# danieleschmidt/DiffFE-Physics-Lab

Hardware: AMD Instinct MI355X
Metric: FEM solves/sec (fwd+adjoint), 2D P1 Poisson 1024^2 mesh, batch=256 per GPU (higher is better)
Workload: dtype f64

## Files before the change

difffe-physics-lab_amd/csrc/lattice.h:

```cpp
#pragma once
#include "common.h"

namespace diffhe_lattice __attribute__((visibility("hidden"))) {

using namespace diffhe;
typedef long long i64;

struct Level {
  int nx, ny, n, W, nd;
  const double* v;
  const float* v32;
  const _Float16* o16;
  const double* osc;
  const float* rd32;
  const float* mk32;
  const unsigned char* bc;
  const void* inv;
  const double* shift;
};

struct h16m {};
template <typename TM> struct MatTypes { typedef TM diag; typedef TM off; };
template <> struct MatTypes<h16m> { typedef float diag; typedef _Float16 off; };
__device__ __forceinline__ double ldc(const double* __restrict__ p, unsigned lv) { return p[lv]; }
__device__ __forceinline__ double ldc(const float* __restrict__ p, unsigned lv) { return (double)p[lv]; }
__device__ __forceinline__ double ldc(const _Float16* __restrict__ p, unsigned lv) { return (double)(float)p[lv]; }

__device__ inline double fast_rcp(double d) {
  const double r0 = __builtin_amdgcn_rcp(d);
  return fma(r0, fma(-d, r0, 1.0), r0);
}

// ... 180 lines not shown
    s.v[3] += (double)p.w;
  }
};

struct Src {
  rsrc_t r;
};
__device__ __forceinline__ Src make_src(const void* p) { return Src{make_rsrc(p)}; }
template <typename VT>
__device__ __forceinline__ VT ldsrc(const Src& s, unsigned voff, unsigned soff) { return VLane<VT>::ld(s.r, voff, soff); }

template <typename VT, bool SHARED> struct Coef;
template <typename VT> struct Coef<VT, true> {
  typedef float T;
  const float *v0, *v1, *v2, *v3, *rdp;
  __device__ __forceinline__ Coef(const Level& L, i64, unsigned, int) : v0(L.v32), v1(L.v32 + L.n), v2(L.v32 + 2 * (i64)L.n),
                                                                        v3(L.v32 + 3 * (i64)L.n), rdp(L.rd32) {}
  __device__ __forceinline__ T d(i64 i) const { return v0[i]; }
  __device__ __forceinline__ T e(i64 i) const { return v1[i]; }
  __device__ __forceinline__ T n2(i64 i) const { return v2[i]; }
  __device__ __forceinline__ T q3(i64 i) const { return v3[i]; }
  __device__ __forceinline__ T rd(i64 i, T) const { return rdp[i]; }
};
__device__ __forceinline__ float ldh(rsrc_t r, unsigned voff, float) {
  return (float)__builtin_bit_cast(_Float16, __builtin_amdgcn_raw_buffer_load_b16(r, voff, 0, 0));
}
__device__ __forceinline__ v2f ldh(rsrc_t r, unsigned voff, v2f) {
  typedef _Float16 h2 __attribute__((ext_vector_type(2)));
  const h2 h = __builtin_bit_cast(h2, __builtin_amdgcn_raw_buffer_load_b32(r, voff, 0, 0));
  return v2f{(float)h.x, (float)h.y};
}
__device__ __forceinline__ unsigned ldraw(rsrc_t r, unsigned voff, float) {
  return (unsigned)(unsigned short)__builtin_amdgcn_raw_buffer_load_b16(r, voff, 0, 0);
}
__device__ __forceinline__ unsigned ldraw(rsrc_t r, unsigned voff, v2f) {
  return (unsigned)__builtin_amdgcn_raw_buffer_load_b32(r, voff, 0, 0);
}
__device__ __forceinline__ float unraw(unsigned raw, float) { return (float)__builtin_bit_cast(_Float16, (unsigned short)raw); }
__device__ __forceinline__ v2f unraw(unsigned raw, v2f) {
  typedef _Float16 h2 __attribute__((ext_vector_type(2)));
  const h2 h = __builtin_bit_cast(h2, raw);
  return v2f{(float)h.x, (float)h.y};
}
template <typename VT> struct Coef<VT, false> {
  typedef VT T;
  rsrc_t r0, r1, r2, r3;
// ... 88 lines not shown
```

difffe-physics-lab_amd/csrc/lattice.hip:

```cpp
#include <stdlib.h>
#include <type_traits>
#include <string.h>

#include "lattice.h"

namespace diffhe_lattice __attribute__((visibility("hidden"))) {
namespace {

__global__ __launch_bounds__(256) void dia_apply_dot_kernel(Level L, int Bv, const double* __restrict__ scale,
                                                             const double* __restrict__ x, double* __restrict__ y,
                                                             double* __restrict__ part, int Bp) {
  __shared__ double lds[4 * kWave];
  const NodeMap nm = node_map(Bp);
  const int vb = Bv == 1 ? 0 : nm.b;
  double s = 0.0;
  for (int i = nm.node0; i < L.n; i += nm.stride) {
    const i64 o = (i64)i * Bp + nm.b;
    const double acc = row_scale(L, scale, i, nm.b) * dia_row(L, Bv, vb, x, i, nm.b, Bp) + shift_at(L, i) * x[o];
    y[o] = acc;
    s += acc * x[o];
  }
  STORE_PARTIAL(part, s);
}

// ... 1144 lines not shown
  if (launches) *launches = g_kp.n[id];
  return DIFFHE_OK;
}

static int fill_hier(Hier& H, const diffhe_mg_level* levels, int n_levels, int Bv, int Bp, const double* scale,
                     const double* omegas, int nu, int n_coarse) {
  if (!levels || n_levels < 1 || n_levels > kMaxLevels) return DIFFHE_E_BADARG;
  if (!diffhe::valid_batch_pad(Bp)) return DIFFHE_E_BATCHPAD;
  if (Bv != 1 && Bv != Bp) return DIFFHE_E_BADARG;
  if (nu < 1 || nu > 8 || n_coarse < 1 || !omegas) return DIFFHE_E_BADARG;
  for (int l = 0; l < n_levels; ++l) {
    const diffhe_mg_level& s = levels[l];
    if (s.nx < 2 || s.ny < 2 || (s.nd != 3 && s.nd != 4) || !s.vals || !s.is_bc) return DIFFHE_E_BADARG;
    if (l > 0) {
      const bool hx = levels[l - 1].nx == 2 * s.nx, hy = levels[l - 1].ny == 2 * s.ny;
      const bool kx = levels[l - 1].nx == s.nx, ky = levels[l - 1].ny == s.ny;
      if (!((hx && hy) || (hx && ky) || (kx && hy))) return DIFFHE_E_BADARG;
    }
    if ((long long)(s.nx + 1) * (s.ny + 1) > 0x7fffffffLL) return DIFFHE_E_TOOBIG;
    Level& L = H.lev[l];
    L.nx = s.nx; L.ny = s.ny; L.W = s.nx + 1; L.n = (s.nx + 1) * (s.ny + 1); L.nd = s.nd;
    L.v = s.vals; L.v32 = s.vals32; L.bc = s.is_bc; L.inv = s.dense_inv; L.shift = s.shift; L.rd32 = s.rdiag32; L.mk32 = s.mask32; L.o16 = (Bv == Bp && Bp > 1 && s.offdiag_scales) ? (const _Float16*)s.offdiag16 : nullptr;
    L.osc = s.offdiag_scales;
  }
  H.nl = n_levels; H.Bv = Bv; H.Bp = Bp; H.scale = scale; H.nu = nu; H.n_coarse = n_coarse;
  H.coarse_lmax = 2.0;
  H.fmg_coarse_cycles = 1;
  H.fuse = Bp % (2 * kWave) == 0 ? 2 : 1;
  H.pre4 = 1;
  H.dense_mfma = 1;
  for (int k = 0; k < 8; ++k) H.omega[k] = omegas[k < nu ? k : nu - 1];
  return DIFFHE_OK;
}

static long long carve(Hier& H, double* work, bool fp32) {
  long long off = 0;
  auto take = [&](long long cnt) {
    if (fp32) cnt = (cnt + 1) / 2;
    cnt = (cnt + 7) & ~7LL;
    double* p = work ? work + off : nullptr;
    off += cnt;
    return (void*)p;
  };
  for (int l = 0; l < H.nl; ++l) {
    const long long nb = (long long)H.lev[l].n * H.Bp;
    H.xa[l] = take(nb);
// ... 382 lines not shown
```

difffe-physics-lab_amd/csrc/lattice_fused.hip:

```cpp
#include "lattice.h"

namespace diffhe_lattice __attribute__((visibility("hidden"))) {
namespace {

template <typename VT, int ND, int CW, bool EDGE, bool SHARED>
__device__ __forceinline__ void fused_pre_body(const Level& L, VT ib, VT sb, const float* __restrict__ rhs,
                                               float* __restrict__ x2out, float* __restrict__ crhs, float w0, float w1,
                                               int cW, const unsigned char* __restrict__ cbc, int Bp, unsigned lb, int c0w,
                                               int r0, int r1) {
  constexpr int RW = 2 * CW + 1;
  constexpr int N1 = RW + 4, N2 = RW + 2;
  const int W = L.W, nyp = L.ny + 1;
  const i64 n = L.n;
  const VT Z = VLane<VT>::zero();
  typedef Coef<VT, SHARED> CF;
  i64 cbase = (i64)(r0 - 3) * W;
  if (cbase < 0) cbase = 0;
  const CF cf(L, cbase, lb, Bp);
  bool ok1[N1];
  unsigned off1[N1];
#pragma unroll
  for (int j = 0; j < N1; ++j) {
    int c = c0w - 2 + j;
    ok1[j] = !EDGE || (c >= 0 && c < W);
    if (EDGE) c = c < 0 ? 0 : (c > W - 1 ? W - 1 : c);
    off1[j] = 4u * ((unsigned)(c - (c0w - 2) + 2) * (unsigned)Bp + lb);
  }
  const i64 tile0 = ((i64)(r0 - 2) * W + (c0w - 4)) * Bp;
  const Src rr = make_src(rhs + tile0);
  const unsigned rowB = 4u * (unsigned)W * (unsigned)Bp;
  const float inv_w0 = 1.0f / w0;

  auto x1_row = [&](int R, VT* dst) {
    if (EDGE && (R < 0 || R >= nyp)) {
#pragma unroll
      for (int j = 0; j < N1; ++j) dst[j] = Z;
      return;
    }
    const unsigned sx = (unsigned)(R - (r0 - 2)) * rowB;
    const i64 rb = (i64)R * W + (c0w - 2);
// ... 230 lines not shown
template <typename VT, int ND, int CW, bool SHARED, int NW = 4, int MW = (SHARED ? 4 : 1)>
__global__ __launch_bounds__(64 * NW, MW) void fused_pre_kernel(Level L, const double* __restrict__ scale,
                                                         const float* __restrict__ rhs, float* __restrict__ x2out,
                                                         float* __restrict__ crhs, float w0, float w1, int cW,
                                                         const unsigned char* __restrict__ cbc, int Bp, int ncb, int TR) {
  constexpr int SPL = VLane<VT>::kSpl;
  const int lane = threadIdx.x & 63;
  const int wave = __builtin_amdgcn_readfirstlane(threadIdx.x >> 6);
  const unsigned lb = blockIdx.y * (SPL * kWave) + SPL * lane;
  const int tile = xcd_tile(blockIdx.x, gridDim.x);
  const int rc = tile / ncb, cb = tile - rc * ncb;
  const int nyp = L.ny + 1;
  const int J0 = (cb * NW + wave) * CW, I0 = rc * TR;
  const int cnyp = (nyp + 1) >> 1;
  const int I1 = (I0 + TR < cnyp) ? I0 + TR : cnyp;
  if (!(J0 < cW && I0 < I1)) return;
  const int c0w = 2 * J0 - 1;
  const int r0 = I0 > 0 ? 2 * I0 - 1 : 0;
  const int r1 = (2 * I1 < nyp) ? 2 * I1 : nyp;
  const VT sb = VLane<VT>::from_scale(scale, lb);
  const VT ib = 1.0f / sb;
  constexpr int RW = 2 * CW + 1;
  const bool edge = c0w - 2 < 0 || c0w + RW + 1 > L.W - 1 || r0 - 2 < 0 || r1 + 1 > nyp - 1;
  if (edge) fused_pre_body<VT, ND, CW, true, SHARED>(L, ib, sb, rhs, x2out, crhs, w0, w1, cW, cbc, Bp, lb, c0w, r0, r1);
  else fused_pre_body<VT, ND, CW, false, SHARED>(L, ib, sb, rhs, x2out, crhs, w0, w1, cW, cbc, Bp, lb, c0w, r0, r1);
}

template <typename VT, int ND, int RW, bool EDGE, bool DOT, bool SHARED, bool XZ>
__device__ __forceinline__ void fused_post_body(const Level& L, VT ib, const float* __restrict__ xin,
                                                const float* __restrict__ rhs, const float* __restrict__ ec,
                                                float* __restrict__ zout, float wA, float wB, int cW, int Bp, unsigned lb,
                                                int c0w, int r0, int r1, Acc& acc) {
  constexpr int N1 = RW + 4, N2 = RW + 2;
  constexpr int NCE = RW / 2 + 3;
  const int W = L.W, nyp = L.ny + 1;
  const i64 n = L.n;
  const VT Z = VLane<VT>::zero();
  typedef Coef<VT, SHARED> CF;
  i64 cbase = (i64)(r0 - 3) * W;
  if (cbase < 0) cbase = 0;
  const CF cf(L, cbase, lb, Bp);
  bool ok1[N1];
  unsigned off1[N1];
#pragma unroll
  for (int j = 0; j < N1; ++j) {
    int c = c0w - 2 + j;
    ok1[j] = !EDGE || (c >= 0 && c < W);
    if (EDGE) c = c < 0 ? 0 : (c > W - 1 ? W - 1 : c);
    off1[j] = 4u * ((unsigned)(c - (c0w - 2) + 2) * (unsigned)Bp + lb);
  }
  const int cj0 = (c0w >> 1) - 1;
  unsigned offc[NCE];
#pragma unroll
  for (int j = 0; j < NCE; ++j) {
    int cj = cj0 + j;
    cj = cj < 0 ? 0 : (cj > cW - 1 ? cW - 1 : cj);
    offc[j] = 4u * ((unsigned)cj * (unsigned)Bp + lb);
  }
  const i64 tile0 = ((i64)(r0 - 2) * W + (c0w - 4)) * Bp;
  const Src rx = make_src(XZ ? rhs + tile0 : xin + tile0);
  const Src rr = make_src(rhs + tile0);
  const int cr0 = (r0 - 2 > 0 ? r0 - 2 : 0) >> 1;
  const Src rc = make_src(ec + (i64)cr0 * cW * Bp);
// ... 3 lines not shown
    if (EDGE && (R < 0 || R >= nyp)) {
#pragma unroll
      for (int j = 0; j < N1; ++j) dst[j] = Z;
      return;
    }
    const unsigned sx = (unsigned)(R - (r0 - 2)) * rowB;
    const unsigned sc = (unsigned)((R >> 1) - cr0) * rowCB;
    VT ce[NCE], ce2[NCE];
#pragma unroll
    for (int j = 0; j < NCE; ++j) {
      ce[j] = ldsrc<VT>(rc, offc[j], sc);
      ce2[j] = (R & 1) ? ldsrc<VT>(rc, offc[j], sc + rowCB) : Z;
    }
    const i64 rb = (i64)R * W + (c0w - 2);
#pragma unroll
    for (int j = 0; j < N1; ++j) {
      VT corr;
      if (!(j & 1))
        corr = (R & 1) ? 0.5f * (ce[j / 2] + ce2[j / 2]) : ce[j / 2];
      else
        corr = (R & 1) ? 0.5f * (ce[(j + 1) / 2] + ce2[(j - 1) / 2]) : 0.5f * (ce[(j - 1) / 2] + ce[(j + 1) / 2]);
      i64 i = rb + j;
      if (EDGE) i = i < 0 ? 0 : (i > n - 1 ? n - 1 : i);
      const VT v = XZ ? L.mk32[i] * corr : ldsrc<VT>(rx, off1[j], sx) + L.mk32[i] * corr;
      dst[j] = ok1[j] ? v : Z;
    }
  };
  auto bu_row = [&](int R, VT* dst) {
    if (EDGE && (R < 0 || R >= nyp)) {
#pragma unroll
      for (int j = 0; j < N2; ++j) dst[j] = Z;
      return;
    }
    const unsigned sx = (unsigned)(R - (r0 - 2)) * rowB;
#pragma unroll
    for (int j = 0; j < N2; ++j) dst[j] = ok1[j + 1] ? ldsrc<VT>(rr, off1[j + 1], sx) * ib : Z;
  };
  auto x3_row = [&](int R, const VT* am, const VT* ac, const VT* ap, const VT* bu, VT* dst) {
    if (EDGE && (R < 0 || R >= nyp)) {
#pragma unroll
      for (int j = 0; j < N2; ++j) dst[j] = Z;
      return;
    }
    k1_row<VT, N2, ND, EDGE>(cf, n, W, R, c0w - 1, am, ac, ap, [&](int j, VT kx, typename CF::T, typename CF::T rd) {
      const VT v = ac[j + 1] + (wA * rd) * (bu[j] - kx);
      dst[j] = ok1[j + 1] ? v : Z;
    });
// ... 119 lines not shown
template <typename VT, int ND, int RW, bool DOT, bool SHARED, bool XZ = false, int NW = 4, int MW = (SHARED ? 4 : 1)>
__global__ __launch_bounds__(64 * NW, MW) void fused_post_kernel(Level L, const double* __restrict__ scale,
                                                          const float* __restrict__ xin, const float* __restrict__ rhs,
                                                          const float* __restrict__ ec, float* __restrict__ zout, float wA,
                                                          float wB, int cW, double* __restrict__ part, int Bp, int ncb,
                                                          int TR) {
  __shared__ double lds[NW * kWave];
  constexpr int SPL = VLane<VT>::kSpl;
  const int lane = threadIdx.x & 63;
  const int wave = __builtin_amdgcn_readfirstlane(threadIdx.x >> 6);
  const unsigned lb = blockIdx.y * (SPL * kWave) + SPL * lane;
  const int tile = xcd_tile(blockIdx.x, gridDim.x);
  const int rc = tile / ncb, cb = tile - rc * ncb;
  const int nyp = L.ny + 1;
  const int c0w = (cb * NW + wave) * RW;
  const int r0 = rc * TR;
  const int r1 = (r0 + TR < nyp) ? r0 + TR : nyp;
  const bool active = c0w < L.W && r0 < r1;
  const VT sb = VLane<VT>::from_scale(scale, lb);
  const VT ib = 1.0f / sb;
  Acc acc;
  if (active) {
    const bool edge = c0w - 2 < 0 || c0w + RW + 1 > L.W - 1 || r0 - 2 < 0 || r1 + 1 > nyp - 1;
    if (edge)
      fused_post_body<VT, ND, RW, true, DOT, SHARED, XZ>(L, ib, xin, rhs, ec, zout, wA, wB, cW, Bp, lb, c0w, r0, r1, acc);
    else
      fused_post_body<VT, ND, RW, false, DOT, SHARED, XZ>(L, ib, xin, rhs, ec, zout, wA, wB, cW, Bp, lb, c0w, r0, r1, acc);
  }
  if (DOT) {
#pragma unroll
    for (int q = 0; q < SPL; ++q) {
      const double f = scale ? scale[lb + q] : 1.0;
      const double t = block_sum_waves<NW>(acc.v[q] * f, lds);
      if (wave == 0) part[(i64)blockIdx.x * Bp + lb + q] = t;
    }
  }
}

}

void launch_fused_pre(const Level& L, const Level& C, int Bv, const double* scale, const float* rhs, float* x2, float* crhs,
                      double w0, double w1, int Bp, const StripGeom& g, int spl, hipStream_t st) {
  constexpr int CW = kRestrictCols;
  diffhe::account((9.0 + (Bv == 1 ? 0.0 : 4.0 + 2.0 * (L.nd - 1))) * (double)L.n * Bp);
  const dim3 grid(g.ncb * g.nrc, Bp / (spl * kWave));
#define FPRE(VT_, ND_, SH_)                                                                                               \
  hipLaunchKernelGGL((fused_pre_kernel<VT_, ND_, CW, SH_>), grid, dim3(256), 0, st, L, scale, rhs, x2, crhs,              \
                     (float)w0, (float)w1, C.W, C.bc, Bp, g.ncb, g.TR)
  if (Bv != 1) { if (L.nd == 3) FPRE(v2f, 3, false); else FPRE(v2f, 4, false); }
// ... 38 lines not shown
```

difffe-physics-lab_amd/diffhe/_hip.py:

```python
from __future__ import annotations

import ctypes as C
import os

import torch

_HERE = os.path.dirname(os.path.abspath(__file__))
LIB_PATH = os.environ.get("DIFFHE_HIP_LIB", os.path.join(os.path.dirname(_HERE), "lib", "libdiffhe_hip.so"))

_P, _I, _L, _D = C.c_void_p, C.c_int, C.c_longlong, C.c_double
ABI_VERSION = 8


class MgLevel(C.Structure):
    _fields_ = [("nx", _I), ("ny", _I), ("nd", _I), ("reserved", _I), ("vals", _P), ("is_bc", _P), ("vals32", _P),
                ("dense_inv", _P), ("shift", _P), ("rdiag32", _P), ("mask32", _P), ("offdiag16", _P), ("offdiag_scales", _P)]


_LV = C.POINTER(MgLevel)


class AmgLevel(C.Structure):
    _fields_ = [("n", _I), ("W", _I), ("vals", _P), ("cols", _P), ("agg", _P), ("agg_ptr", _P), ("agg_members", _P),
                ("vals32", _P), ("agg_weights", _P), ("p_cols", _P), ("p_vals", _P), ("p_width", _I), ("reserved", _I),
                ("dense_inv", _P)]


_AV = C.POINTER(AmgLevel)


class _Ptr:
    dtype = None

    @classmethod
    def from_param(cls, v):
        if v is None:
            return None
        if type(v) is int:
# ... 163 lines not shown
```

difffe-physics-lab_amd/diffhe/plan.py:

```python
from __future__ import annotations

import collections
import hashlib
import os
import shutil
import threading
from typing import Optional

import numpy as np
import torch

from . import _hip


_TLS = threading.local()


def status_buffer() -> torch.Tensor:
    buf = getattr(_TLS, "status", None)
    if buf is None:
        buf = _TLS.status = torch.zeros(4, dtype=torch.int32).pin_memory()
    return buf


# ... 284 lines not shown
    k0[~keep] = 0.0
    Mref = np.array([[6, -1, -1, 0, -4, 0], [-1, 6, -1, 0, 0, -4], [-1, -1, 6, -4, 0, 0],
                     [0, 0, -4, 32, 16, 16], [-4, 0, 0, 16, 32, 16], [0, -4, 0, 16, 16, 32]], dtype=np.float64) / 180.0
    m0 = Mref[None] * np.where(keep, area, 0.0)[:, None, None]
    return (np.ascontiguousarray(k0.reshape(-1, 36).T), np.ascontiguousarray(m0.reshape(-1, 36).T))


def _lumped_mass(nodes: np.ndarray, elements: np.ndarray) -> np.ndarray:
    n = nodes.shape[0]
    if nodes.shape[1] == 1:
        size = np.abs(nodes[elements[:, 1], 0] - nodes[elements[:, 0], 0])
    elif nodes.shape[1] == 3:
        _, det, keep = _tet_cofactors(np.ascontiguousarray(nodes.T), elements.T.astype(np.int64))
        size = np.where(keep, np.abs(det) / 6.0, 0.0)
    else:
        a, b, c = (nodes[elements[:, k]] for k in range(3))
        size = 0.5 * np.abs((b[:, 0] - a[:, 0]) * (c[:, 1] - a[:, 1]) - (c[:, 0] - a[:, 0]) * (b[:, 1] - a[:, 1]))
    m = np.zeros(n)
    for k in range(elements.shape[1]):
        np.add.at(m, elements[:, k], size / elements.shape[1])
    return m


class LatticeLevel:

    def __init__(self, nodes2d: np.ndarray, is_bc2d: np.ndarray, device, with_load_matrix: bool = False):
        L = _hip.lib()
        ny, nx = nodes2d.shape[0] - 1, nodes2d.shape[1] - 1
        self.nx, self.ny = nx, ny
        self.n, self.m = (nx + 1) * (ny + 1), 2 * nx * ny
        dev = lambda a: torch.from_numpy(np.ascontiguousarray(a)).to(device)
        self.coords = dev(nodes2d.reshape(self.n, 2).T)
        self.elems = dev(lattice_elements(nx, ny).T.astype(np.int32))
        self.is_bc = dev(is_bc2d.reshape(self.n).astype(np.uint8))
        pat = host_arrays(f"dia_{nx}x{ny}", lambda: build_dia_pattern(nx, ny))
        self.cols, self.ent_ptr, self.contrib = dev(pat["cols"]), dev(pat["ent_ptr"]), dev(pat["contrib"])
        self.k0 = torch.empty((9, self.m), dtype=torch.float64, device=device)
        m0 = torch.empty((9, self.m), dtype=torch.float64, device=device)
        L.diffhe_p1_element_integrals(self.coords, self.elems, 2, self.n, self.m, self.k0, m0, _stream(device))
        self._m0 = m0 if with_load_matrix else None
        flat = np.ascontiguousarray(nodes2d.reshape(self.n, 2).T)
        ref = host_arrays(f"refint_{nx}x{ny}_{hashlib.blake2b(flat.tobytes(), digest_size=8).hexdigest()}",
                          lambda: dict(zip(("tn", "dn"), reference_order_integrals(flat, lattice_elements(nx, ny).T))))
        self.tnum, self.den = dev(ref["tn"]), dev(ref["dn"])
        hyp = max(float(self.k0[5, 0::2].abs().max()), float(self.k0[2, 1::2].abs().max()))
        self.nd = 3 if hyp == 0.0 else 4
# ... 119 lines not shown
            self._bc_index = torch.nonzero(self.is_bc).reshape(-1)
        return self._bc_index

    _WARM_MAX = 4

    def warm_get(self, key):
        with self._lock:
            x = self.warm.get(key)
            if x is not None:
                self.warm.move_to_end(key)
            return x

    def warm_put(self, key, x):
        with self._lock:
            self.warm[key] = x
            self.warm.move_to_end(key)
            while len(self.warm) > self._WARM_MAX:
                self.warm.popitem(last=False)

    def shared_fp32(self, vals, cacheable: bool):
        key = len(vals)
        cache = self.__dict__.setdefault("_fp32_cache", {})
        if cacheable and key in cache:
            return cache[key]
        v32 = [v.float() for v in vals]
        rd32 = [(1.0 / v[0]).float().contiguous() for v in vals]
        if cacheable:
            with self._lock:
                cache[key] = (v32, rd32)
        return v32, rd32

    def dense_level(self, max_nodes: int = 1200):
        return next((i for i, lev in enumerate(self.levels) if lev.n <= max_nodes), None)

    def dense_coarse(self, idx: int, vals, fp32: bool):
        key = (idx, bool(fp32))
        cache = self.__dict__.setdefault("_dense_cache", {})
        with self._lock:
            self._dense_coarse_build(cache, key, idx, vals, fp32)
        return idx, cache[key]

    def _dense_coarse_build(self, cache, key, idx, vals, fp32):
        if key not in cache:
            lev = self.levels[idx]
            d = vals[idx].detach().to("cpu", torch.float64).numpy().reshape(lev.nd, lev.n)
            n, W = lev.n, lev.nx + 1
            K = np.zeros((n, n))
            i = np.arange(n)
            K[i, i] = d[0]
            for k, off in ((1, 1), (2, W)) + (((3, lev.nx),) if lev.nd == 4 else ()):
                j = i[: n - off]
                K[j, j + off] = d[k][: n - off]
                K[j + off, j] = d[k][: n - off]
# ... 278 lines not shown
```

difffe-physics-lab_amd/diffhe/solver.py:

```python
from __future__ import annotations

import ctypes
import itertools
import math
import os
import threading
import warnings
import weakref
from dataclasses import dataclass, replace
from typing import Dict, NamedTuple, Optional, Tuple

import torch
import torch.nn as nn

from . import _hip
from .mesh import FEMesh
from .plan import SolvePlan, get_plan, padded_batch, status_buffer, _stream

K_SCALAR, K_SAMPLE, K_ELEM, K_SAMPLE_ELEM = 0, 1, 2, 3


@dataclass
class SolveInfo:
    path: str = ""
    iterations: int = 0
    not_converged: int = 0
    max_relres: float = 0.0
    adj_iterations: int = 0
    adj_max_relres: float = 0.0
    err_est: float = 0.0
    adj_err_est: float = 0.0
    stop_rules: Optional[dict] = None
    adj_stop_rules: Optional[dict] = None
    tol_energy: float = 0.0
    coeff_storage: str = ""
    factored: bool = False
    flags: int = 0
    precision: str = ""
    hierarchy: str = ""
    hierarchy_levels: int = 0
    operator_complexity: float = 0.0
    hierarchy_age: int = 0


def _resolve_device(device) -> torch.device:
    if device is not None:
        device = torch.device(device)
        if device.type != "cuda":
            raise RuntimeError("diffhe runs on a ROCm GPU only (no CPU fallback)")
        return device
    if not torch.cuda.is_available():
        raise RuntimeError("diffhe: no ROCm GPU visible -- the HIP solve path has no CPU fallback")
    return torch.device("cuda", torch.cuda.current_device())


def _kappa_mode(kappa: torch.Tensor, m: int, B: Optional[int]):
    if kappa.numel() == 1:
        return K_SCALAR, None
    if kappa.dim() == 1:
        if kappa.shape[0] == m and (B is None or B == 1 or B != m):
            return K_ELEM, None
# ... 12 lines not shown
        return K_SCALAR, None, False
    if kappa.dim() == 2 and shape[1] == nc:
        if shape[0] == m and (B is None or B == 1 or B != m):
            return K_ELEM, None, False
        return K_SAMPLE, shape[0], False
    if kappa.dim() == 3:
        if node_major and B is not None and shape == (nc, m, B):
            return K_SAMPLE_ELEM, B, True
        if shape[1:] == (m, nc):
            return K_SAMPLE_ELEM, shape[0], False
    raise ValueError(f"conductivity tensor shape {shape} not understood for a mesh with {m} elements: expected "
                     f"({nc},), ({m}, {nc}), (B, {nc}) or (B, {m}, {nc}) in Voigt components"
                     + (f", or ({nc}, {m}, B) with layout='node'" if node_major else ""))


class _Solved(NamedTuple):
    x: torch.Tensor
    iterations: int
    not_converged: int
    relres: torch.Tensor
    est: Optional[torch.Tensor] = None
    rule: Optional[torch.Tensor] = None
    flags: int = 0


class _Engine:

    def __init__(self, plan: SolvePlan, tol: float, max_iter: int, check_every: int, assembly: str, *,
                 ref_order: bool = False, g: Optional[torch.Tensor] = None):
        self.p = plan
        self.tol, self.max_iter, self.check_every, self.assembly = tol, max_iter, check_every, assembly
        self.ref_order = ref_order
        self.g = plan.g if g is None else g
        self.L = _hip.lib()

    def to_node_major(self, src, B, Bp, n, zero_mask=None):
        p = self.p
        dst = torch.empty((n, Bp), dtype=torch.float64, device=p.device)
        ld = 0 if src.dim() == 1 else src.stride(0)
        self.L.diffhe_to_node_major(src, ld, zero_mask, dst, n, B, Bp, _stream(p.device))
        return dst

    def to_sample_major(self, src, B, Bp, n, add=None):
        p = self.p
        dst = torch.empty((B, n), dtype=torch.float64, device=p.device)
        self.L.diffhe_to_sample_major(src, add, dst, n, n, B, Bp, _stream(p.device))
# ... 198 lines not shown
        lev0 = (_hip.MgLevel * 1)()
        lev0[0].nx, lev0[0].ny, lev0[0].nd = p.levels[0].nx, p.levels[0].ny, p.levels[0].nd
        lev0[0].vals, lev0[0].is_bc = vals[0].data_ptr(), p.levels[0].is_bc.data_ptr()
        dmax = torch.empty(Bv, dtype=torch.float64, device=p.device)
        L.diffhe_lattice_max_diag(lev0, Bv, dmax, st)
        mant, expo = torch.frexp(dmax)
        scales = torch.ldexp(torch.ones_like(dmax), expo - (mant == 0.5).to(expo.dtype))
        ok = torch.isfinite(dmax) & (dmax > 0)
        scales = torch.where(ok, scales, torch.ones_like(scales)).contiguous()
        flags = torch.zeros(1, dtype=torch.int32, device=p.device)
        d32, o16 = [], []
        for lev, v in zip(p.levels, vals):
            one = (_hip.MgLevel * 1)()
            one[0].nx, one[0].ny, one[0].nd, one[0].vals = lev.nx, lev.ny, lev.nd, v.data_ptr()
            d = torch.empty((lev.n, Bv), dtype=torch.float32, device=p.device)
            o = torch.empty((lev.nd - 1, lev.n, Bv), dtype=torch.float16, device=p.device)
            L.diffhe_lattice_pack_h16(one, Bv, scales, d, o, flags, st)
            d32.append(d)
            o16.append(o)
        if not bool(ok.all()) or int(flags[0]) != 0:
            return None, None, None
        return d32, o16, scales

    def lattice_levels(self, vals, vals32=None, dense=None, shift=None, rdiag32=None, off16=None):
        off16, oscales = off16 if off16 is not None else (None, None)
        nl = len(vals) if dense is None else dense[0] + 1
        arr = (_hip.MgLevel * nl)()
        for i, (lev, v) in enumerate(zip(self.p.levels[:nl], vals[:nl])):
            arr[i].nx, arr[i].ny, arr[i].nd, arr[i].reserved = lev.nx, lev.ny, lev.nd, 0
            arr[i].vals, arr[i].is_bc = v.data_ptr(), lev.is_bc.data_ptr()
            arr[i].vals32 = vals32[i].data_ptr() if vals32 is not None and vals32[i] is not None else None
            arr[i].dense_inv = dense[1].data_ptr() if dense is not None and i == nl - 1 else None
            arr[i].shift = shift[i].data_ptr() if shift is not None else None
            arr[i].rdiag32 = rdiag32[i].data_ptr() if rdiag32 is not None and rdiag32[i] is not None else None
            arr[i].offdiag16 = off16[i].data_ptr() if off16 is not None and off16[i] is not None else None
            arr[i].mask32 = lev.mask32().data_ptr() if (arr[i].rdiag32 or arr[i].offdiag16) else None
            arr[i].offdiag_scales = oscales.data_ptr() if arr[i].offdiag16 else None
        return arr

    def lattice_pcg(self, vals, Bv, scale, rhs, Bp, mg, vals32=None, dense=None, x0=None, shift=None, rdiag32=None,
                    off16=None):
        p, L = self.p, self.L
        arr = self.lattice_levels(vals, vals32, dense, shift, rdiag32, off16)
        nl = len(arr)
        warm = x0 is not None and x0.shape == (p.n, Bp)
        work = torch.empty(L.diffhe_lattice_pcg_workspace_doubles(arr, nl, Bp), dtype=torch.float64, device=p.device)
        omegas = mg.get("omegas") or ([0.56, 1.39] if mg["nu"] == 2 else [mg["omega"]] * mg["nu"])
        om = (ctypes.c_double * len(omegas))(*omegas)
        est = torch.empty(Bp, dtype=torch.float64, device=p.device)
        rule = torch.empty(Bp, dtype=torch.int32, device=p.device)
        closed_step = (p.closed_boundary and p.regular_cells and p.dense_level() is not None
                       and int(mg.get("cg_fp32_steplength", 1)))
        flags = (int(mg.get("fp32", 0)) * _hip.PCG_FP32 | int(mg.get("fmg", 0)) * _hip.PCG_FMG
                 | ((int(mg.get("fmg_cycles", 1)) - 1) << _hip.PCG_FMG_CYCLES_SHIFT)
                 | (0 if int(mg.get("floor", 1)) else _hip.PCG_NO_FLOOR)
                 | (_hip.PCG_WARM if warm else 0)
                 | (0 if int(mg.get("fused", 1)) else _hip.PCG_UNFUSED)
                 | (0 if int(mg.get("dense_mfma", 1)) else _hip.PCG_DENSE_SCALAR)
                 | (0 if int(mg.get("pre4", 1)) else _hip.PCG_PRE2)
                 | (0 if int(mg.get("resid_pair", 1)) else _hip.PCG_RESID_FP64)
                 | (_hip.PCG_CLOSED_FP32_STEP if closed_step else 0))
        return self._solve(Bp, lambda x, relres, iters, st: L.diffhe_lattice_pcg_solve(
            arr, nl, Bv, scale, rhs, x, Bp, self.tol, float(mg.get("tol_energy", 0.0) or 0.0), min(self.max_iter, 500),
            len(omegas), mg["n_coarse"], om, flags, work, relres, est, iters, rule, st, _stream(p.device)),
            x=x0.clone() if warm else None, est=est, rule=rule, flags=flags)

    def amg_setup(self, vals, Bv, fp32=True, levels=None, dense_coarse=False):
        p, L = self.p, self.L
        st = _stream(p.device)
        chain = [dict(n=p.n, W=p.W, vals=vals, cols=p.cols)]
        for lv in (levels if levels is not None else p.amg_levels):
            vc = torch.empty((lv["W"], lv["n"], Bv), dtype=torch.float64, device=p.device)
            L.diffhe_ell_galerkin(chain[-1]["vals"], lv["ent_ptr"], lv["contrib"], lv.get("weights"), vc, lv["n"],
                                  lv["W"], Bv, st)
            chain[-1].update(agg=lv["agg"], agg_ptr=lv["agg_ptr"], agg_members=lv["agg_members"],
                             agg_weights=lv.get("agg_weights"), p_cols=lv.get("p_cols"), p_vals=lv.get("p_vals"))
            if "lam_parent" in lv:
                chain[-1]["lam"] = lv["lam_parent"]
            chain.append(dict(n=lv["n"], W=lv["W"], vals=vc, cols=lv["cols"], lam=lv.get("lam")))
        arr = (_hip.AmgLevel * len(chain))()
        for i, lv in enumerate(chain):
            arr[i].n, arr[i].W = lv["n"], lv["W"]
            arr[i].vals, arr[i].cols = lv["vals"].data_ptr(), lv["cols"].data_ptr()
            if lv.get("lam"):
                arr[i].reserved = int(math.ceil(1000.0 * lv["lam"]))
            if fp32 and Bv != 1:
                lv["vals32"] = lv["vals"].to(torch.float32)
                arr[i].vals32 = lv["vals32"].data_ptr()
# ... 426 lines not shown
        info.path = "lattice-mgpcg"
        Bp = self.Bp = padded_batch(B)
        self.kappa_value = call.kappa.detach().to(plan.device, torch.float64).reshape(-1)[0] if mode == K_SCALAR else None
        closed_ = plan.closed_boundary and solver.operator != "assembled"
        self.factored = factored = closed_ and mode in (K_SCALAR, K_SAMPLE)
        didx = plan.dense_level() if (factored and self.mg.get("dense_coarse", 1) and reaction == 0.0) else None
        vals, Bv, scale, lift, lift_scale = eng.lattice_assemble(call.kappa, mode, B, Bp, factor=closed_,
                                                                 n_levels=None if didx is None else didx + 1,
                                                                 em=call.kappa_em)
        self.shift = eng.reaction_shifts(reaction, len(vals)) if reaction and factored else None
        if reaction and not factored:
            eng.add_reaction(vals, reaction, lattice=True)
        rhs = self._rhs(call, lift, Bv, lift_scale)
        self.vals32, self.rdiag32, self.off16 = self._cycle_coeffs(vals, Bv)
        info.coeff_storage = ("fp64" if not self.mg.get("fp32") else
                              ("fp16-rowsum" if self.off16 is not None else "fp32") if Bv != 1 else "shared-fp32")
        self.direct, self.dense = didx == 0, None
        if didx is not None:
            if self.direct:
                info.path = "lattice-direct"
                self.mg = dict(self.mg, fp32=0)
            self.dense = plan.dense_coarse(didx, vals, bool(self.mg.get("fp32")))
        self.wkey = (Bp, mode, reaction)
        x, its, bad, relres, est, rule, flags = eng.lattice_pcg(
            vals, Bv, scale, rhs, Bp, self.mg, self.vals32, self.dense,
            x0=plan.warm_get(("u",) + self.wkey) if solver.warm_start else None, shift=self.shift, rdiag32=self.rdiag32,
            off16=self.off16)
        if solver.warm_start and not bad:
            shares = call.node_major and Bp == B and not plan.has_dirichlet_data and call.bc is None
            plan.warm_put(("u",) + self.wkey, x.clone() if shares else x)
        info.stop_rules = _rule_counts(rule, B) if not self.direct else {}
        info.flags = flags
        info.precision = _precision_text(flags, info.coeff_storage, Bv, Bp, int(eng.L.diffhe_lattice_fused_passes()),
                                         bool(eng.L.diffhe_lattice_recompute_ap()))
        info.tol_energy = float(self.mg.get("tol_energy", 0.0) or 0.0)
        info.factored = bool(factored)
        info.iterations, info.not_converged = its, bad
        info.max_relres = float(relres[:B].max())
        info.err_est = float(est[:B].max())
        self.vals, self.x, self.Bv, self.scale = vals, x, Bv, scale
        self.lift = lift if Bv == 1 else None
        return _from_node_major(eng, x, B, Bp, plan.n, call.node_major, call.bc)

    def _cycle_coeffs(self, vals, Bv):
        mg, Bp = self.mg, self.Bp
        vals32 = rdiag32 = off16 = None
        if mg.get("fp32") and Bv != 1 and mg.get("h16", 1) and Bp > 1:
            d32_, o16_, osc_ = self.eng.pack_cycle_coeffs(vals, Bv)
            if d32_ is not None:
                vals32, off16 = d32_, (o16_, osc_)
        if mg.get("fp32") and Bv != 1 and vals32 is None:
            vals32 = [v.float() for v in vals]
        elif mg.get("fp32") and Bv == 1 and mg.get("strip2", 1) and Bp % 64 == 0 and self.shift is None:
            vals32, rdiag32 = self.plan.shared_fp32(vals, cacheable=self.factored)
        return vals32, rdiag32, off16
# ... 419 lines not shown
        if assembly not in ("gather", "atomic"):
            raise ValueError(f"Unknown assembly: {assembly!r}")
        if method not in ("auto", "ell", "ell-jacobi"):
            raise ValueError(f"Unknown method: {method!r}")
        if chain not in ("reference", "exact"):
            raise ValueError(f"Unknown chain mode: {chain!r}")
        if operator not in ("auto", "assembled"):
            raise ValueError(f"Unknown operator: {operator!r}")
        self.operator = operator
        self.chain = chain
        if not (float(reaction) >= 0.0):
            raise ValueError(f"reaction must be >= 0, got {reaction!r}")
        self.reaction = float(reaction)
        if warm_start not in (False, True, "forward"):
            raise ValueError(f"Unknown warm_start: {warm_start!r}")
        self.warm_start = warm_start
        self.method = method
        self.amg = dict(n_coarse=16, gamma=None, scale=None, fp32=0, max_iter=20000, smoothed=1)
        for item in filter(None, os.environ.get("DIFFHE_AMG", "").split(",")):
            key, val = item.split("=")
            self.amg[key] = float(val) if key in ("scale", "strength") else int(val)
        self.amg.update(amg or {})
        self._amg_user = set((amg or {}).keys()) | {i.split("=")[0] for i in os.environ.get("DIFFHE_AMG", "").split(",") if i}
        self.mg = dict(nu=2, n_coarse=8, omega=0.8, omegas=None, fp32=1, fmg=1, floor=1, tol_energy=1e-11)
        for item in filter(None, os.environ.get("DIFFHE_MG", "").split(",")):
            key, val = item.split("=")
            if key == "omegas":
                self.mg[key] = [float(v) for v in val.split(":")]
            else:
                self.mg[key] = float(val) if key in ("omega", "tol_energy") else int(val)
        self.mg.update(mg or {})
        self._mg_user = set((mg or {}).keys()) | {i.split("=")[0] for i in os.environ.get("DIFFHE_MG", "").split(",") if i}
        self._device = device
        if os.environ.get("DIFFHE_TOL"):
            tol = float(os.environ["DIFFHE_TOL"])
        self._tol_user = tol
        self.tol, self.max_iter, self.check_every, self.assembly = tol, max_iter, check_every, assembly
        self.last_info = SolveInfo()
        self._hier_lock = threading.Lock()
        self._hier_cache: Dict[tuple, dict] = {}

    def refresh_hierarchy(self) -> None:
        with self._hier_lock:
            self._hier_cache.clear()

    def _hierarchy_levels(self, plan: SolvePlan, theta: float, refresh: int, build):
        key = (id(plan), float(theta), True)
# ... 115 lines not shown
```

include/diffhe_hip.h:

```cpp
#ifndef DIFFHE_HIP_H
#define DIFFHE_HIP_H

#ifdef __cplusplus
extern "C" {
#endif

#define DIFFHE_ABI_VERSION 8

#define DIFFHE_OK 0
#define DIFFHE_E_BADARG (-1)
#define DIFFHE_E_LAUNCH (-2)
#define DIFFHE_E_TOOBIG (-3)
#define DIFFHE_E_BATCHPAD (-4)

int diffhe_abi_version(void);
const char* diffhe_status_string(int status);
const char* diffhe_last_hip_error(void);

int diffhe_traffic_account(int reset, double* bytes_host, long long* launches_host);

#define DIFFHE_CHAIN_REFERENCE_ORDER 1

long long diffhe_chain1d_stage_doubles(int n, int B, int max_seg_len, int flags);

// ... 51 lines not shown
  const float* vals32;
  const double* agg_weights;
  const int* p_cols;
  const double* p_vals;
  int p_width;
  int reserved;
  const double* dense_inv;
} diffhe_amg_level;

int diffhe_ell_galerkin(const double* vals_fine, const int* ent_ptr, const int* contrib, const double* weights,
                        double* vals_coarse, int n_coarse, int W_coarse, int Bv, void* stream);
long long diffhe_ell_amg_workspace_doubles(const diffhe_amg_level* levels, int n_levels, int Bp);
int diffhe_ell_amg_pcg_solve(const diffhe_amg_level* levels, int n_levels, int Bv, const double* b, double* x, int Bp,
                             double tol, int max_iter, int n_coarse, int gamma, double scale, int flags,
                             double* work,
                             double* relres, int* iters, int* status_host, void* stream);

int diffhe_ell_apply(const double* vals, const int* cols, const double* x, double* y, double* part, int n, int W,
                     int Bp, int Bv, void* stream);

typedef struct diffhe_mg_level {
  int nx, ny;
  int nd;
  int reserved;
  const double* vals;
  const unsigned char* is_bc;
  const float* vals32;
  const void* dense_inv;
  const double* shift;
  const float* rdiag32;
  const float* mask32;
  const void* offdiag16;
  const double* offdiag_scales;
} diffhe_mg_level;

#define DIFFHE_PCG_FP32 1
#define DIFFHE_PCG_FMG 2
#define DIFFHE_PCG_FMG_CYCLES_SHIFT 2
#define DIFFHE_PCG_NO_FLOOR 16
#define DIFFHE_PCG_WARM 32
#define DIFFHE_PCG_UNFUSED 64
#define DIFFHE_PCG_DENSE_SCALAR 128
#define DIFFHE_PCG_CLOSED_FP32_STEP 256
#define DIFFHE_PCG_PRE2 512
#define DIFFHE_PCG_RESID_FP64 (1 << 10)

long long diffhe_lattice_pcg_workspace_doubles(const diffhe_mg_level* levels, int n_levels, int Bp);
// ... 110 lines not shown
```

Measured before the change: 3283.

## Use uniform scalar stencil coefficients for interior tiles in fused smoother kernels

The host now detects, per multigrid level, an interior margin beyond which the fp32 stencil coefficients, reciprocal diagonal and mask are all constant, and passes it through the previously reserved struct field. Fused pre/post smoother kernels check whether a tile lies entirely inside that margin and, if so, instantiate a variant that loads the coefficients once as scalars and drops the per-node coefficient and mask loads. This targets memory traffic from coefficient arrays in the shared-coefficient, 3-diagonal case. It adds host-side checks on every cached level, extra template instantiations with possible code-size and register pressure, and depends on the operator being spatially uniform.

```diff
diff --git a/difffe-physics-lab_amd/csrc/lattice.h b/difffe-physics-lab_amd/csrc/lattice.h
--- a/difffe-physics-lab_amd/csrc/lattice.h
+++ b/difffe-physics-lab_amd/csrc/lattice.h
@@ -8,6 +8,7 @@
 
 struct Level {
   int nx, ny, n, W, nd;
+  int uni;
   const double* v;
   const float* v32;
   const _Float16* o16;
@@ -234,6 +235,21 @@
   __device__ __forceinline__ T q3(i64 i) const { return v3[i]; }
   __device__ __forceinline__ T rd(i64 i, T) const { return rdp[i]; }
 };
+template <typename VT> struct CoefUni {
+  typedef float T;
+  float dv, ev, nv, rdv;
+  __device__ __forceinline__ CoefUni(const Level& L, i64 i0, unsigned, int)
+      : dv(L.v32[i0]), ev(L.v32[L.n + i0]), nv(L.v32[2 * (i64)L.n + i0]), rdv(L.rd32[i0]) {}
+  __device__ __forceinline__ T d(i64) const { return dv; }
+  __device__ __forceinline__ T e(i64) const { return ev; }
+  __device__ __forceinline__ T n2(i64) const { return nv; }
+  __device__ __forceinline__ T q3(i64) const { return 0.0f; }
+  __device__ __forceinline__ T rd(i64, T) const { return rdv; }
+};
+__host__ __device__ inline bool tile_in_margin(const Level& L, int rlo, int rhi, int clo, int chi) {
+  const int m = L.uni;
+  return m > 0 && rlo >= m && rhi <= L.ny - m && clo >= m && chi <= L.nx - m;
+}
 __device__ __forceinline__ float ldh(rsrc_t r, unsigned voff, float) {
   return (float)__builtin_bit_cast(_Float16, __builtin_amdgcn_raw_buffer_load_b16(r, voff, 0, 0));
 }
diff --git a/difffe-physics-lab_amd/csrc/lattice.hip b/difffe-physics-lab_amd/csrc/lattice.hip
--- a/difffe-physics-lab_amd/csrc/lattice.hip
+++ b/difffe-physics-lab_amd/csrc/lattice.hip
@@ -1190,6 +1190,8 @@
     L.nx = s.nx; L.ny = s.ny; L.W = s.nx + 1; L.n = (s.nx + 1) * (s.ny + 1); L.nd = s.nd;
     L.v = s.vals; L.v32 = s.vals32; L.bc = s.is_bc; L.inv = s.dense_inv; L.shift = s.shift; L.rd32 = s.rdiag32; L.mk32 = s.mask32; L.o16 = (Bv == Bp && Bp > 1 && s.offdiag_scales) ? (const _Float16*)s.offdiag16 : nullptr;
     L.osc = s.offdiag_scales;
+    if (s.uniform_margin < 0) return DIFFHE_E_BADARG;
+    L.uni = shared32_ok(L, Bv, Bp) ? s.uniform_margin : 0;
   }
   H.nl = n_levels; H.Bv = Bv; H.Bp = Bp; H.scale = scale; H.nu = nu; H.n_coarse = n_coarse;
   H.coarse_lmax = 2.0;
diff --git a/difffe-physics-lab_amd/csrc/lattice_fused.hip b/difffe-physics-lab_amd/csrc/lattice_fused.hip
--- a/difffe-physics-lab_amd/csrc/lattice_fused.hip
+++ b/difffe-physics-lab_amd/csrc/lattice_fused.hip
@@ -3,7 +3,7 @@
 namespace diffhe_lattice __attribute__((visibility("hidden"))) {
 namespace {
 
-template <typename VT, int ND, int CW, bool EDGE, bool SHARED>
+template <typename VT, int ND, int CW, bool EDGE, bool SHARED, bool UNI = false>
 __device__ __forceinline__ void fused_pre_body(const Level& L, VT ib, VT sb, const float* __restrict__ rhs,
                                                float* __restrict__ x2out, float* __restrict__ crhs, float w0, float w1,
                                                int cW, const unsigned char* __restrict__ cbc, int Bp, unsigned lb, int c0w,
@@ -13,9 +13,10 @@
   const int W = L.W, nyp = L.ny + 1;
   const i64 n = L.n;
   const VT Z = VLane<VT>::zero();
-  typedef Coef<VT, SHARED> CF;
+  typedef std::conditional_t<UNI, CoefUni<VT>, Coef<VT, SHARED>> CF;
   i64 cbase = (i64)(r0 - 3) * W;
   if (cbase < 0) cbase = 0;
+  if (UNI) cbase = (i64)(r0 - 2) * W + (c0w - 2);
   const CF cf(L, cbase, lb, Bp);
   bool ok1[N1];
   unsigned off1[N1];
@@ -292,11 +293,17 @@
   const VT ib = 1.0f / sb;
   constexpr int RW = 2 * CW + 1;
   const bool edge = c0w - 2 < 0 || c0w + RW + 1 > L.W - 1 || r0 - 2 < 0 || r1 + 1 > nyp - 1;
+  bool uni = false;
+  if constexpr (SHARED && ND == 3) uni = !edge && tile_in_margin(L, r0 - 2, r1 + 1, c0w - 2, c0w + RW + 1);
   if (edge) fused_pre_body<VT, ND, CW, true, SHARED>(L, ib, sb, rhs, x2out, crhs, w0, w1, cW, cbc, Bp, lb, c0w, r0, r1);
-  else fused_pre_body<VT, ND, CW, false, SHARED>(L, ib, sb, rhs, x2out, crhs, w0, w1, cW, cbc, Bp, lb, c0w, r0, r1);
-}
-
-template <typename VT, int ND, int RW, bool EDGE, bool DOT, bool SHARED, bool XZ>
+  else if constexpr (SHARED && ND == 3) {
+    if (uni) fused_pre_body<VT, ND, CW, false, SHARED, true>(L, ib, sb, rhs, x2out, crhs, w0, w1, cW, cbc, Bp, lb, c0w, r0, r1);
+    else fused_pre_body<VT, ND, CW, false, SHARED>(L, ib, sb, rhs, x2out, crhs, w0, w1, cW, cbc, Bp, lb, c0w, r0, r1);
+  } else
+    fused_pre_body<VT, ND, CW, false, SHARED>(L, ib, sb, rhs, x2out, crhs, w0, w1, cW, cbc, Bp, lb, c0w, r0, r1);
+}
+
+template <typename VT, int ND, int RW, bool EDGE, bool DOT, bool SHARED, bool XZ, bool UNI = false>
 __device__ __forceinline__ void fused_post_body(const Level& L, VT ib, const float* __restrict__ xin,
                                                 const float* __restrict__ rhs, const float* __restrict__ ec,
                                                 float* __restrict__ zout, float wA, float wB, int cW, int Bp, unsigned lb,
@@ -306,9 +313,10 @@
   const int W = L.W, nyp = L.ny + 1;
   const i64 n = L.n;
   const VT Z = VLane<VT>::zero();
-  typedef Coef<VT, SHARED> CF;
+  typedef std::conditional_t<UNI, CoefUni<VT>, Coef<VT, SHARED>> CF;
   i64 cbase = (i64)(r0 - 3) * W;
   if (cbase < 0) cbase = 0;
+  if (UNI) cbase = (i64)(r0 - 2) * W + (c0w - 2);
   const CF cf(L, cbase, lb, Bp);
   bool ok1[N1];
   unsigned off1[N1];
@@ -358,7 +366,9 @@
         corr = (R & 1) ? 0.5f * (ce[(j + 1) / 2] + ce2[(j - 1) / 2]) : 0.5f * (ce[(j - 1) / 2] + ce[(j + 1) / 2]);
       i64 i = rb + j;
       if (EDGE) i = i < 0 ? 0 : (i > n - 1 ? n - 1 : i);
-      const VT v = XZ ? L.mk32[i] * corr : ldsrc<VT>(rx, off1[j], sx) + L.mk32[i] * corr;
+      VT v;
+      if (UNI) v = XZ ? corr : ldsrc<VT>(rx, off1[j], sx) + corr;
+      else v = XZ ? L.mk32[i] * corr : ldsrc<VT>(rx, off1[j], sx) + L.mk32[i] * corr;
       dst[j] = ok1[j] ? v : Z;
     }
   };
@@ -524,9 +534,16 @@
   Acc acc;
   if (active) {
     const bool edge = c0w - 2 < 0 || c0w + RW + 1 > L.W - 1 || r0 - 2 < 0 || r1 + 1 > nyp - 1;
+    bool uni = false;
+    if constexpr (SHARED && ND == 3) uni = !edge && tile_in_margin(L, r0 - 2, r1 + 1, c0w - 2, c0w + RW + 1);
     if (edge)
       fused_post_body<VT, ND, RW, true, DOT, SHARED, XZ>(L, ib, xin, rhs, ec, zout, wA, wB, cW, Bp, lb, c0w, r0, r1, acc);
-    else
+    else if constexpr (SHARED && ND == 3) {
+      if (uni)
+        fused_post_body<VT, ND, RW, false, DOT, SHARED, XZ, true>(L, ib, xin, rhs, ec, zout, wA, wB, cW, Bp, lb, c0w, r0, r1, acc);
+      else
+        fused_post_body<VT, ND, RW, false, DOT, SHARED, XZ>(L, ib, xin, rhs, ec, zout, wA, wB, cW, Bp, lb, c0w, r0, r1, acc);
+    } else
       fused_post_body<VT, ND, RW, false, DOT, SHARED, XZ>(L, ib, xin, rhs, ec, zout, wA, wB, cW, Bp, lb, c0w, r0, r1, acc);
   }
   if (DOT) {
diff --git a/difffe-physics-lab_amd/diffhe/_hip.py b/difffe-physics-lab_amd/diffhe/_hip.py
--- a/difffe-physics-lab_amd/diffhe/_hip.py
+++ b/difffe-physics-lab_amd/diffhe/_hip.py
@@ -13,7 +13,7 @@
 
 
 class MgLevel(C.Structure):
-    _fields_ = [("nx", _I), ("ny", _I), ("nd", _I), ("reserved", _I), ("vals", _P), ("is_bc", _P), ("vals32", _P),
+    _fields_ = [("nx", _I), ("ny", _I), ("nd", _I), ("uniform_margin", _I), ("vals", _P), ("is_bc", _P), ("vals32", _P),
                 ("dense_inv", _P), ("shift", _P), ("rdiag32", _P), ("mask32", _P), ("offdiag16", _P), ("offdiag_scales", _P)]
 
 
diff --git a/difffe-physics-lab_amd/diffhe/plan.py b/difffe-physics-lab_amd/diffhe/plan.py
--- a/difffe-physics-lab_amd/diffhe/plan.py
+++ b/difffe-physics-lab_amd/diffhe/plan.py
@@ -330,6 +330,22 @@
     return m
 
 
+UNIFORM_MARGIN_MAX = 4
+
+
+def uniform_margin(v32: torch.Tensor, rd32: torch.Tensor, mask32: torch.Tensor, cap: int = UNIFORM_MARGIN_MAX) -> int:
+    ny, nx = rd32.shape[0] - 1, rd32.shape[1] - 1
+    for m in range(1, cap + 1):
+        if ny - m < m or nx - m < m:
+            break
+        v = v32[:, m:ny - m + 1, m:nx - m + 1]
+        r = rd32[m:ny - m + 1, m:nx - m + 1]
+        if (bool((v == v[:, :1, :1]).all()) and bool((r == r[:1, :1]).all())
+                and bool((mask32[m:ny - m + 1, m:nx - m + 1] == 1.0).all())):
+            return m
+    return 0
+
+
 class LatticeLevel:
 
     def __init__(self, nodes2d: np.ndarray, is_bc2d: np.ndarray, device, with_load_matrix: bool = False):
@@ -495,13 +511,22 @@
         key = len(vals)
         cache = self.__dict__.setdefault("_fp32_cache", {})
         if cacheable and key in cache:
-            return cache[key]
+            return cache[key][:2]
         v32 = [v.float() for v in vals]
         rd32 = [(1.0 / v[0]).float().contiguous() for v in vals]
         if cacheable:
+            margins = [uniform_margin(v.reshape(lev.nd, lev.ny + 1, lev.nx + 1), r.reshape(lev.ny + 1, lev.nx + 1),
+                                      lev.mask32().reshape(lev.ny + 1, lev.nx + 1))
+                       for lev, v, r in zip(self.levels, v32, rd32)]
             with self._lock:
-                cache[key] = (v32, rd32)
+                cache[key] = (v32, rd32, margins)
         return v32, rd32
+
+    def shared_margins(self, rdiag32):
+        for _, rd32, margins in self.__dict__.get("_fp32_cache", {}).values():
+            if rd32 is rdiag32:
+                return margins
+        return None
 
     def dense_level(self, max_nodes: int = 1200):
         return next((i for i, lev in enumerate(self.levels) if lev.n <= max_nodes), None)
diff --git a/difffe-physics-lab_amd/diffhe/solver.py b/difffe-physics-lab_amd/diffhe/solver.py
--- a/difffe-physics-lab_amd/diffhe/solver.py
+++ b/difffe-physics-lab_amd/diffhe/solver.py
@@ -37,6 +37,7 @@
     factored: bool = False
     flags: int = 0
     precision: str = ""
+    uniform_margins: Optional[list] = None
     hierarchy: str = ""
     hierarchy_levels: int = 0
     operator_complexity: float = 0.0
@@ -95,6 +96,7 @@
     est: Optional[torch.Tensor] = None
     rule: Optional[torch.Tensor] = None
     flags: int = 0
+    margins: Optional[list] = None
 
 
 class _Engine:
@@ -339,12 +341,12 @@
             return None, None, None
         return d32, o16, scales
 
-    def lattice_levels(self, vals, vals32=None, dense=None, shift=None, rdiag32=None, off16=None):
+    def lattice_levels(self, vals, vals32=None, dense=None, shift=None, rdiag32=None, off16=None, margins=None):
         off16, oscales = off16 if off16 is not None else (None, None)
         nl = len(vals) if dense is None else dense[0] + 1
         arr = (_hip.MgLevel * nl)()
         for i, (lev, v) in enumerate(zip(self.p.levels[:nl], vals[:nl])):
-            arr[i].nx, arr[i].ny, arr[i].nd, arr[i].reserved = lev.nx, lev.ny, lev.nd, 0
+            arr[i].nx, arr[i].ny, arr[i].nd, arr[i].uniform_margin = lev.nx, lev.ny, lev.nd, 0
             arr[i].vals, arr[i].is_bc = v.data_ptr(), lev.is_bc.data_ptr()
             arr[i].vals32 = vals32[i].data_ptr() if vals32 is not None and vals32[i] is not None else None
             arr[i].dense_inv = dense[1].data_ptr() if dense is not None and i == nl - 1 else None
@@ -353,12 +355,15 @@
             arr[i].offdiag16 = off16[i].data_ptr() if off16 is not None and off16[i] is not None else None
             arr[i].mask32 = lev.mask32().data_ptr() if (arr[i].rdiag32 or arr[i].offdiag16) else None
             arr[i].offdiag_scales = oscales.data_ptr() if arr[i].offdiag16 else None
+            if margins is not None and arr[i].rdiag32 and arr[i].vals32 and shift is None:
+                arr[i].uniform_margin = int(margins[i])
         return arr
 
     def lattice_pcg(self, vals, Bv, scale, rhs, Bp, mg, vals32=None, dense=None, x0=None, shift=None, rdiag32=None,
                     off16=None):
         p, L = self.p, self.L
-        arr = self.lattice_levels(vals, vals32, dense, shift, rdiag32, off16)
+        margins = p.shared_margins(rdiag32) if rdiag32 is not None and Bv == 1 and int(mg.get("uniform", 1)) else None
+        arr = self.lattice_levels(vals, vals32, dense, shift, rdiag32, off16, margins)
         nl = len(arr)
         warm = x0 is not None and x0.shape == (p.n, Bp)
         work = torch.empty(L.diffhe_lattice_pcg_workspace_doubles(arr, nl, Bp), dtype=torch.float64, device=p.device)
@@ -380,7 +385,8 @@
         return self._solve(Bp, lambda x, relres, iters, st: L.diffhe_lattice_pcg_solve(
             arr, nl, Bv, scale, rhs, x, Bp, self.tol, float(mg.get("tol_energy", 0.0) or 0.0), min(self.max_iter, 500),
             len(omegas), mg["n_coarse"], om, flags, work, relres, est, iters, rule, st, _stream(p.device)),
-            x=x0.clone() if warm else None, est=est, rule=rule, flags=flags)
+            x=x0.clone() if warm else None, est=est, rule=rule, flags=flags,
+            margins=[int(a.uniform_margin) for a in arr])
 
     def amg_setup(self, vals, Bv, fp32=True, levels=None, dense_coarse=False):
         p, L = self.p, self.L
@@ -853,7 +859,7 @@
                 self.mg = dict(self.mg, fp32=0)
             self.dense = plan.dense_coarse(didx, vals, bool(self.mg.get("fp32")))
         self.wkey = (Bp, mode, reaction)
-        x, its, bad, relres, est, rule, flags = eng.lattice_pcg(
+        x, its, bad, relres, est, rule, flags, margins = eng.lattice_pcg(
             vals, Bv, scale, rhs, Bp, self.mg, self.vals32, self.dense,
             x0=plan.warm_get(("u",) + self.wkey) if solver.warm_start else None, shift=self.shift, rdiag32=self.rdiag32,
             off16=self.off16)
@@ -862,6 +868,7 @@
             plan.warm_put(("u",) + self.wkey, x.clone() if shares else x)
         info.stop_rules = _rule_counts(rule, B) if not self.direct else {}
         info.flags = flags
+        info.uniform_margins = margins
         info.precision = _precision_text(flags, info.coeff_storage, Bv, Bp, int(eng.L.diffhe_lattice_fused_passes()),
                                          bool(eng.L.diffhe_lattice_recompute_ap()))
         info.tol_energy = float(self.mg.get("tol_energy", 0.0) or 0.0)
@@ -1327,7 +1334,7 @@
             self.amg[key] = float(val) if key in ("scale", "strength") else int(val)
         self.amg.update(amg or {})
         self._amg_user = set((amg or {}).keys()) | {i.split("=")[0] for i in os.environ.get("DIFFHE_AMG", "").split(",") if i}
-        self.mg = dict(nu=2, n_coarse=8, omega=0.8, omegas=None, fp32=1, fmg=1, floor=1, tol_energy=1e-11)
+        self.mg = dict(nu=2, n_coarse=8, omega=0.8, omegas=None, fp32=1, fmg=1, floor=1, tol_energy=1e-11, uniform=1)
         for item in filter(None, os.environ.get("DIFFHE_MG", "").split(",")):
             key, val = item.split("=")
             if key == "omegas":
diff --git a/include/diffhe_hip.h b/include/diffhe_hip.h
--- a/include/diffhe_hip.h
+++ b/include/diffhe_hip.h
@@ -97,7 +97,7 @@
 typedef struct diffhe_mg_level {
   int nx, ny;
   int nd;
-  int reserved;
+  int uniform_margin;
   const double* vals;
   const unsigned char* is_bc;
   const float* vals32;
```

Result: no change. 3254 (-0.9%).
